# Advaith-Sajeev/LiDAR-Vision-VQA

Hardware: NVIDIA B200
Metric: lidar_encoder_sweeps_per_sec (higher is better)
Workload: dtype f32

## Files before the change

### lidar_vision_vqa_b200/csrc/scatter.cu

```cuda
#include <cuda_fp16.h>

#include <cstdlib>

#include "common.cuh"

namespace pillars {

namespace {

constexpr int kThreads = 256;

__global__ void k_build_cell_row(const void *__restrict__ coords, int coords_float, int64_t m,
                                 const int32_t *__restrict__ m_dev, int nb, int nx, int ny, int nz,
                                 int32_t *__restrict__ cell_row)
{
    const int64_t i = static_cast<int64_t>(blockIdx.x) * blockDim.x + threadIdx.x;
    int64_t live = m;
    if (m_dev) live = tmin<int64_t>(m, static_cast<int64_t>(*m_dev));
    if (i >= live) return;
    int b, z, y, x;
    if (coords_float) {
        const float4 c = *reinterpret_cast<const float4 *>(static_cast<const float *>(coords) + i * 4);
        b = static_cast<int>(c.x); z = static_cast<int>(c.y); y = static_cast<int>(c.z); x = static_cast<int>(c.w);
    } else {
        const int4 c = *reinterpret_cast<const int4 *>(static_cast<const int32_t *>(coords) + i * 4);
        b = c.x; z = c.y; y = c.z; x = c.w;
    }
    const int64_t plane = static_cast<int64_t>(nx) * ny * nz;
    const int64_t cell = nz > 1 ? (static_cast<int64_t>(z) * ny + y) * nx + x : static_cast<int64_t>(z) + static_cast<int64_t>(y) * nx + x;
    if (b < 0 || b >= nb || cell < 0 || cell >= plane || x < 0 || x >= nx) return;
    atomicMax(cell_row + static_cast<int64_t>(b) * plane + cell, static_cast<int32_t>(i));
}

__global__ void k_rebase_segments(int32_t *__restrict__ coords, int n_seg, int64_t rows_per_seg, int64_t seg_stride,
                                  const int32_t *__restrict__ seg_counts, int64_t count_stride, int frames_per_seg,
                                  int32_t *__restrict__ overflow)
{
    const int64_t i = static_cast<int64_t>(blockIdx.x) * blockDim.x + threadIdx.x;
    if (i >= rows_per_seg * n_seg) return;
    const int seg = static_cast<int>(i / rows_per_seg);
    const int64_t r = i - seg * rows_per_seg;
    const int32_t cnt = __ldg(seg_counts + static_cast<int64_t>(seg) * count_stride);
    int32_t *b = coords + seg * seg_stride + r * 4;
    if (r < cnt) *b += seg * frames_per_seg;
    else *b = -1;
    if (r == 0 && cnt > rows_per_seg && overflow) *overflow = 1;
}

template <bool VEC, int CPP, bool PIPE>
__global__ void __launch_bounds__(kThreads)
k_scatter_plain(const float *__restrict__ feats, const int32_t *__restrict__ cell_row, int f, int64_t plane,
                int tiles_per_plane, float *__restrict__ bev)
{
    constexpr int kPer = VEC ? 4 : 1;
    const int b = blockIdx.x / tiles_per_plane;
    const int64_t cell0 = static_cast<int64_t>(blockIdx.x % tiles_per_plane) * (blockDim.x * kPer) + threadIdx.x * kPer;
    const bool inb = cell0 < plane;
    int32_t r[kPer];
#pragma unroll
    for (int k = 0; k < kPer; ++k) r[k] = -1;
    if (inb) {
        if (VEC) {
            const int4 v = __ldg(reinterpret_cast<const int4 *>(cell_row + b * plane + cell0));
            r[0] = v.x; r[1 % kPer] = v.y; r[2 % kPer] = v.z; r[3 % kPer] = v.w;
        } else {
            r[0] = __ldg(cell_row + b * plane + cell0);
        }
    }
    bool any = false;
#pragma unroll
    for (int k = 0; k < kPer; ++k) any |= r[k] >= 0;
    float *dst = bev + (static_cast<int64_t>(b) * f) * plane + cell0;
    if (!__any_sync(0xffffffffu, any)) {
        if (inb) {
            if (VEC) {
#pragma unroll 8
                for (int c = 0; c < f; ++c) __stcs(reinterpret_cast<float4 *>(dst + c * plane), make_float4(0.f, 0.f, 0.f, 0.f));
            } else {
                for (int c = 0; c < f; ++c) __stcs(dst + c * plane, 0.f);
            }
        }
        return;
    }
    if (!inb) return;
    if (VEC) {
        constexpr int kV = CPP / 4;
        float4 cur[4][kV], nxt[4][kV];
        auto fetch = [&](float4 (&dstv)[4][kV], int c0) {
#pragma unroll
            for (int k = 0; k < 4; ++k) {
#pragma unroll
                for (int q = 0; q < kV; ++q) dstv[k][q] = make_float4(0.f, 0.f, 0.f, 0.f);
                if (r[k % kPer] >= 0) {
                    const float4 *row = reinterpret_cast<const float4 *>(feats + static_cast<int64_t>(r[k % kPer]) * f + c0);
#pragma unroll
                    for (int q = 0; q < kV; ++q) dstv[k][q] = __ldg(row + q);
                }
            }
        };
        fetch(cur, 0);
        for (int c0 = 0; c0 < f; c0 += CPP) {
            if (PIPE && c0 + CPP < f) fetch(nxt, c0 + CPP);
#pragma unroll
            for (int q = 0; q < kV; ++q) {
                __stcs(reinterpret_cast<float4 *>(dst + (c0 + 4 * q + 0) * plane), make_float4(cur[0][q].x, cur[1][q].x, cur[2][q].x, cur[3][q].x));
                __stcs(reinterpret_cast<float4 *>(dst + (c0 + 4 * q + 1) * plane), make_float4(cur[0][q].y, cur[1][q].y, cur[2][q].y, cur[3][q].y));
                __stcs(reinterpret_cast<float4 *>(dst + (c0 + 4 * q + 2) * plane), make_float4(cur[0][q].z, cur[1][q].z, cur[2][q].z, cur[3][q].z));
                __stcs(reinterpret_cast<float4 *>(dst + (c0 + 4 * q + 3) * plane), make_float4(cur[0][q].w, cur[1][q].w, cur[2][q].w, cur[3][q].w));
            }
            if (c0 + CPP < f) {
                if (PIPE) {
#pragma unroll
                    for (int k = 0; k < 4; ++k)
#pragma unroll
                        for (int q = 0; q < kV; ++q) cur[k][q] = nxt[k][q];
                } else {
                    fetch(cur, c0 + CPP);
                }
            }
        }
    } else {
        for (int c = 0; c < f; ++c) __stcs(dst + c * plane, r[0] >= 0 ? __ldg(feats + static_cast<int64_t>(r[0]) * f + c) : 0.f);
    }
}

__host__ __device__ __forceinline__ int64_t occ_words(int64_t plane) { return (plane + 255) >> 8; }

__device__ __forceinline__ uint32_t occ_prev_word(const uint32_t *__restrict__ occ_prev, int64_t plane, int tiles_per_plane,
                                                  int groups, int tile_major)
{
    if (!occ_prev) return 0xffffffffu;
    const int tile = tile_major ? (blockIdx.x / groups) % tiles_per_plane : blockIdx.x % tiles_per_plane;
    const int b = blockIdx.x / (groups * tiles_per_plane);
    const int64_t word = (static_cast<int64_t>(tile) * blockDim.x + threadIdx.x) >> 5;
    return word < occ_words(plane) ? __ldg(occ_prev + b * occ_words(plane) + word) : 0xffffffffu;
}

__device__ __forceinline__ void stg256(float *p, float a, float b, float c, float d, float e, float f, float g, float h)
{
    asm volatile("st.global.L1::no_allocate.v8.f32 [%0], {%1, %2, %3, %4, %5, %6, %7, %8};" ::"l"(p), "f"(a), "f"(b), "f"(c),
                 "f"(d), "f"(e), "f"(f), "f"(g), "f"(h)
                 : "memory");
}
__device__ __forceinline__ void stg256_cs(float *p, float a, float b, float c, float d, float e, float f, float g, float h)
{
    asm volatile("st.global.cs.v8.f32 [%0], {%1, %2, %3, %4, %5, %6, %7, %8};" ::"l"(p), "f"(a), "f"(b), "f"(c), "f"(d),
                 "f"(e), "f"(f), "f"(g), "f"(h)
                 : "memory");
}

template <bool CS, int CPP>
__global__ void __launch_bounds__(kThreads)
k_scatter_wide(const float *__restrict__ feats, const int32_t *__restrict__ cell_row, int f, int64_t plane,
               int tiles_per_plane, int chan_per_cta, int tile_major, float *__restrict__ bev,
               const uint32_t *__restrict__ occ_prev, uint32_t *__restrict__ occ_next)
{
    const uint32_t prev = occ_prev_word(occ_prev, plane, tiles_per_plane, f / chan_per_cta, tile_major);
    pdl_wait();
    const int groups = f / chan_per_cta;
    int b, tile, cg;
    if (tile_major) {
        cg = blockIdx.x % groups;
        tile = (blockIdx.x / groups) % tiles_per_plane;
        b = blockIdx.x / (groups * tiles_per_plane);
    } else {
        tile = blockIdx.x % tiles_per_plane;
        cg = (blockIdx.x / tiles_per_plane) % groups;
        b = blockIdx.x / (groups * tiles_per_plane);
    }
    const int64_t cell0 = static_cast<int64_t>(tile) * (blockDim.x * 8) + threadIdx.x * 8;
    const bool inb = cell0 < plane;
    int32_t r[8];
#pragma unroll
    for (int k = 0; k < 8; ++k) r[k] = -1;
    if (inb) {
        const int4 *src = reinterpret_cast<const int4 *>(cell_row + b * plane + cell0);
        const int4 v = __ldg(src), w = __ldg(src + 1);
        r[0] = v.x; r[1] = v.y; r[2] = v.z; r[3] = v.w;
        r[4] = w.x; r[5] = w.y; r[6] = w.z; r[7] = w.w;
    }
    bool any = false;
#pragma unroll
    for (int k = 0; k < 8; ++k) any |= r[k] >= 0;
    const int c_begin = cg * chan_per_cta, c_end = c_begin + chan_per_cta;
    float *dst = bev + (static_cast<int64_t>(b) * f) * plane + cell0;
    auto store = [&](float *p, float a, float b2, float c, float d, float e, float f2, float g, float h) {
        if (CS) stg256_cs(p, a, b2, c, d, e, f2, g, h);
        else stg256(p, a, b2, c, d, e, f2, g, h);
    };
    const uint32_t now = __ballot_sync(0xffffffffu, any);
    if (occ_next && cg == 0 && (threadIdx.x & 31) == 0 && inb) occ_next[b * occ_words(plane) + (cell0 >> 8)] = now;
    if (!inb || !(any || ((prev >> (threadIdx.x & 31)) & 1u))) return;
    if (now == 0) {
#pragma unroll 8
        for (int c = c_begin; c < c_end; ++c) store(dst + c * plane, 0.f, 0.f, 0.f, 0.f, 0.f, 0.f, 0.f, 0.f);
        return;
    }
    constexpr int kV = CPP / 4;
    for (int c0 = c_begin; c0 < c_end; c0 += CPP) {
        float4 v[8][kV];
#pragma unroll
        for (int k = 0; k < 8; ++k) {
#pragma unroll
            for (int q = 0; q < kV; ++q) v[k][q] = make_float4(0.f, 0.f, 0.f, 0.f);
            if (r[k] >= 0) {
                const float4 *row = reinterpret_cast<const float4 *>(feats + static_cast<int64_t>(r[k]) * f + c0);
#pragma unroll
                for (int q = 0; q < kV; ++q) v[k][q] = __ldg(row + q);
            }
        }
#pragma unroll
        for (int q = 0; q < kV; ++q) {
            float *d = dst + (c0 + 4 * q) * plane;
            store(d, v[0][q].x, v[1][q].x, v[2][q].x, v[3][q].x, v[4][q].x, v[5][q].x, v[6][q].x, v[7][q].x);
            store(d + plane, v[0][q].y, v[1][q].y, v[2][q].y, v[3][q].y, v[4][q].y, v[5][q].y, v[6][q].y, v[7][q].y);
            store(d + 2 * plane, v[0][q].z, v[1][q].z, v[2][q].z, v[3][q].z, v[4][q].z, v[5][q].z, v[6][q].z, v[7][q].z);
            store(d + 3 * plane, v[0][q].w, v[1][q].w, v[2][q].w, v[3][q].w, v[4][q].w, v[5][q].w, v[6][q].w, v[7][q].w);
        }
    }
}

__device__ __forceinline__ void ldg256_stream(const float *p, float (&v)[8])
{
    asm volatile("ld.global.nc.L1::no_allocate.v8.f32 {%0, %1, %2, %3, %4, %5, %6, %7}, [%8];"
                 : "=f"(v[0]), "=f"(v[1]), "=f"(v[2]), "=f"(v[3]), "=f"(v[4]), "=f"(v[5]), "=f"(v[6]), "=f"(v[7])
                 : "l"(p));
}

__global__ void __launch_bounds__(kThreads)
k_scatter_wide_half(const float *__restrict__ feats, const int32_t *__restrict__ cell_row, int f, int64_t plane,
                    int tiles_per_plane, __half *__restrict__ bev, const uint32_t *__restrict__ occ_prev,
                    uint32_t *__restrict__ occ_next)
{
    const uint32_t prev = occ_prev_word(occ_prev, plane, tiles_per_plane, f >> 3, 0);
    const int groups = f >> 3;
    const int tile = blockIdx.x % tiles_per_plane;
    const int cg = (blockIdx.x / tiles_per_plane) % groups;
    const int b = blockIdx.x / (groups * tiles_per_plane);
    const int64_t cell0 = static_cast<int64_t>(tile) * (blockDim.x * 8) + threadIdx.x * 8;
    const bool inb = cell0 < plane;
    int32_t r[8];
#pragma unroll
    for (int k = 0; k < 8; ++k) r[k] = -1;
    if (inb) {
        const int4 *src = reinterpret_cast<const int4 *>(cell_row + b * plane + cell0);
        const int4 v = __ldg(src), w = __ldg(src + 1);
        r[0] = v.x; r[1] = v.y; r[2] = v.z; r[3] = v.w;
        r[4] = w.x; r[5] = w.y; r[6] = w.z; r[7] = w.w;
    }
    bool any = false;
#pragma unroll
    for (int k = 0; k < 8; ++k) any |= r[k] >= 0;
    const int c0 = cg * 8;
    __half *dst = bev + (static_cast<int64_t>(b) * f + c0) * plane + cell0;
    const uint32_t now = __ballot_sync(0xffffffffu, any);
    if (occ_next && cg == 0 && (threadIdx.x & 31) == 0 && inb) occ_next[b * occ_words(plane) + (cell0 >> 8)] = now;
    const uint32_t pair = (now | prev) | (((now | prev) >> 1) & 0x55555555u) | (((now | prev) & 0x55555555u) << 1);
    if (!inb || !((pair >> (threadIdx.x & 31)) & 1u)) return;
    if (now == 0) {
#pragma unroll
        for (int c = 0; c < 8; ++c) __stcs(reinterpret_cast<uint4 *>(dst + c * plane), make_uint4(0u, 0u, 0u, 0u));
        return;
    }
    float v[8][8];
#pragma unroll
    for (int k = 0; k < 8; ++k) {
#pragma unroll
        for (int c = 0; c < 8; ++c) v[k][c] = 0.f;
        if (r[k] >= 0) ldg256_stream(feats + static_cast<int64_t>(r[k]) * f + c0, v[k]);
    }
#pragma unroll
    for (int c = 0; c < 8; ++c) {
        uint4 o;
        __half2 h;
        h = __floats2half2_rn(v[0][c], v[1][c]); o.x = *reinterpret_cast<uint32_t *>(&h);
        h = __floats2half2_rn(v[2][c], v[3][c]); o.y = *reinterpret_cast<uint32_t *>(&h);
        h = __floats2half2_rn(v[4][c], v[5][c]); o.z = *reinterpret_cast<uint32_t *>(&h);
        h = __floats2half2_rn(v[6][c], v[7][c]); o.w = *reinterpret_cast<uint32_t *>(&h);
        *reinterpret_cast<uint4 *>(dst + c * plane) = o;
    }
}

}

cudaError_t launch_build_cell_row(const void *coords, bool coords_float, int64_t m, const int32_t *m_dev, int nb, int nx,
                                  int ny, int nz, int32_t *cell_row, cudaStream_t st)
{
    cudaError_t err = cudaMemsetAsync(cell_row, 0xFF, sizeof(int32_t) * static_cast<size_t>(nb) * nx * ny * nz, st);
    note_launch();
    if (err != cudaSuccess || m == 0) return err;
    const unsigned blocks = static_cast<unsigned>((m + kThreads - 1) / kThreads);
    k_build_cell_row<<<blocks, kThreads, 0, st>>>(coords, coords_float ? 1 : 0, m, m_dev, nb, nx, ny, nz, cell_row);
    note_launch();
    return cudaGetLastError();
}

cudaError_t launch_rebase_segments(int32_t *coords, int n_seg, int64_t rows_per_seg, int64_t seg_stride,
                                   const int32_t *seg_counts, int64_t count_stride, int frames_per_seg, int32_t *overflow,
                                   cudaStream_t st)
{
    const int64_t total = rows_per_seg * n_seg;
    if (total == 0) return cudaSuccess;
    k_rebase_segments<<<static_cast<unsigned>((total + kThreads - 1) / kThreads), kThreads, 0, st>>>(
        coords, n_seg, rows_per_seg, seg_stride, seg_counts, count_stride, frames_per_seg, overflow);
    note_launch();
    return cudaGetLastError();
}

cudaError_t launch_scatter_half(const float *feats, const int32_t *cell_row, int nb, int f, int nx, int ny, void *bev,
                                cudaStream_t st, const uint32_t *occ_prev, uint32_t *occ_next)
{
    const int64_t plane = static_cast<int64_t>(nx) * ny;
    if (nb == 0 || plane == 0 || f == 0) return cudaSuccess;
    if (plane % 8 != 0 || f % 8 != 0 || reinterpret_cast<uintptr_t>(bev) % 16 != 0 ||
        reinterpret_cast<uintptr_t>(feats) % 32 != 0)
        return cudaErrorInvalidValue;
    const int bs = 128;
    const int tpp = static_cast<int>((plane + bs * 8 - 1) / (bs * 8));
    const unsigned grid = static_cast<unsigned>(nb) * tpp * (f / 8);
    k_scatter_wide_half<<<grid, bs, 0, st>>>(feats, cell_row, f, plane, tpp, static_cast<__half *>(bev), occ_prev, occ_next);
    note_launch();
    return cudaGetLastError();
}
cudaError_t launch_scatter(const float *feats, const int32_t *cell_row, int nb, int f, int nx, int ny, float *bev,
                           int variant, cudaStream_t st, const uint32_t *occ_prev, uint32_t *occ_next)
{
    const int64_t plane = static_cast<int64_t>(nx) * ny;
    if (nb == 0 || plane == 0 || f == 0) return cudaSuccess;
    const bool vec_ok = (plane % 4 == 0) && (reinterpret_cast<uintptr_t>(bev) % 16 == 0) &&
                        (reinterpret_cast<uintptr_t>(feats) % 16 == 0) && (f % 8 == 0);
    const bool wide_ok = vec_ok && (plane % 8 == 0) && (reinterpret_cast<uintptr_t>(bev) % 32 == 0);
    if (variant != 1 && wide_ok) {
        constexpr int bs = 128, chan = 8;
        const int tpp = static_cast<int>((plane + bs * 8 - 1) / (bs * 8));
        const unsigned grid = static_cast<unsigned>(nb) * tpp * (f / chan);
        static const bool cs = getenv("PILLARS_SCATTER_CS") != nullptr;
        const cudaError_t err = cs ? launch_pdl(k_scatter_wide<true, 8>, dim3(grid), dim3(bs), 0, st, feats, cell_row, f, plane,
                                                tpp, chan, 0, bev, occ_prev, occ_next)
                                   : launch_pdl(k_scatter_wide<false, 8>, dim3(grid), dim3(bs), 0, st, feats, cell_row, f,
                                                plane, tpp, chan, 0, bev, occ_prev, occ_next);
        if (err != cudaSuccess) return err;
        note_launch();
        return cudaGetLastError();
    }
    if (occ_next) {
        const cudaError_t err = cudaMemsetAsync(occ_next, 0xFF, sizeof(uint32_t) * nb * occ_words(plane), st);
        if (err != cudaSuccess) return err;
        note_launch();
    }
    if (vec_ok) {
        const int tpp = static_cast<int>((plane + kThreads * 4 - 1) / (kThreads * 4));
        k_scatter_plain<true, 8, false><<<static_cast<unsigned>(nb) * tpp, kThreads, 0, st>>>(feats, cell_row, f, plane, tpp, bev);
    } else {
        const int tpp = static_cast<int>((plane + kThreads - 1) / kThreads);
        k_scatter_plain<false, 8, false><<<static_cast<unsigned>(nb) * tpp, kThreads, 0, st>>>(feats, cell_row, f, plane, tpp, bev);
    }
    note_launch();
    return cudaGetLastError();
}

}
```

Measured before the change: 89500.

## Add compacted sparse scatter kernel driven by occupancy bitmaps

Adds a sparse scatter kernel that is used whenever a previous occupancy bitmap is available. Each warp reads one bitmap word and ballots which 8-cell groups are occupied now or were occupied before, then compacts those groups into shared memory. The block only loops over that dirty work across all channel chunks, instead of launching a dense grid of tiles per channel group that mostly exit early. The dense kernels drop their occ_prev early-exit logic, and the new kernel adds a shared-memory compaction step plus a block-wide sync.

```diff
diff --git a/lidar_vision_vqa_b200/csrc/scatter.cu b/lidar_vision_vqa_b200/csrc/scatter.cu
--- a/lidar_vision_vqa_b200/csrc/scatter.cu
+++ b/lidar_vision_vqa_b200/csrc/scatter.cu
@@ -126,16 +126,6 @@
 
 __host__ __device__ __forceinline__ int64_t occ_words(int64_t plane) { return (plane + 255) >> 8; }
 
-__device__ __forceinline__ uint32_t occ_prev_word(const uint32_t *__restrict__ occ_prev, int64_t plane, int tiles_per_plane,
-                                                  int groups, int tile_major)
-{
-    if (!occ_prev) return 0xffffffffu;
-    const int tile = tile_major ? (blockIdx.x / groups) % tiles_per_plane : blockIdx.x % tiles_per_plane;
-    const int b = blockIdx.x / (groups * tiles_per_plane);
-    const int64_t word = (static_cast<int64_t>(tile) * blockDim.x + threadIdx.x) >> 5;
-    return word < occ_words(plane) ? __ldg(occ_prev + b * occ_words(plane) + word) : 0xffffffffu;
-}
-
 __device__ __forceinline__ void stg256(float *p, float a, float b, float c, float d, float e, float f, float g, float h)
 {
     asm volatile("st.global.L1::no_allocate.v8.f32 [%0], {%1, %2, %3, %4, %5, %6, %7, %8};" ::"l"(p), "f"(a), "f"(b), "f"(c),
@@ -152,10 +142,8 @@
 template <bool CS, int CPP>
 __global__ void __launch_bounds__(kThreads)
 k_scatter_wide(const float *__restrict__ feats, const int32_t *__restrict__ cell_row, int f, int64_t plane,
-               int tiles_per_plane, int chan_per_cta, int tile_major, float *__restrict__ bev,
-               const uint32_t *__restrict__ occ_prev, uint32_t *__restrict__ occ_next)
-{
-    const uint32_t prev = occ_prev_word(occ_prev, plane, tiles_per_plane, f / chan_per_cta, tile_major);
+               int tiles_per_plane, int chan_per_cta, int tile_major, float *__restrict__ bev, uint32_t *__restrict__ occ_next)
+{
     pdl_wait();
     const int groups = f / chan_per_cta;
     int b, tile, cg;
@@ -190,7 +178,7 @@
     };
     const uint32_t now = __ballot_sync(0xffffffffu, any);
     if (occ_next && cg == 0 && (threadIdx.x & 31) == 0 && inb) occ_next[b * occ_words(plane) + (cell0 >> 8)] = now;
-    if (!inb || !(any || ((prev >> (threadIdx.x & 31)) & 1u))) return;
+    if (!inb) return;
     if (now == 0) {
 #pragma unroll 8
         for (int c = c_begin; c < c_end; ++c) store(dst + c * plane, 0.f, 0.f, 0.f, 0.f, 0.f, 0.f, 0.f, 0.f);
@@ -229,10 +217,8 @@
 
 __global__ void __launch_bounds__(kThreads)
 k_scatter_wide_half(const float *__restrict__ feats, const int32_t *__restrict__ cell_row, int f, int64_t plane,
-                    int tiles_per_plane, __half *__restrict__ bev, const uint32_t *__restrict__ occ_prev,
-                    uint32_t *__restrict__ occ_next)
-{
-    const uint32_t prev = occ_prev_word(occ_prev, plane, tiles_per_plane, f >> 3, 0);
+                    int tiles_per_plane, __half *__restrict__ bev, uint32_t *__restrict__ occ_next)
+{
     const int groups = f >> 3;
     const int tile = blockIdx.x % tiles_per_plane;
     const int cg = (blockIdx.x / tiles_per_plane) % groups;
@@ -255,8 +241,7 @@
     __half *dst = bev + (static_cast<int64_t>(b) * f + c0) * plane + cell0;
     const uint32_t now = __ballot_sync(0xffffffffu, any);
     if (occ_next && cg == 0 && (threadIdx.x & 31) == 0 && inb) occ_next[b * occ_words(plane) + (cell0 >> 8)] = now;
-    const uint32_t pair = (now | prev) | (((now | prev) >> 1) & 0x55555555u) | (((now | prev) & 0x55555555u) << 1);
-    if (!inb || !((pair >> (threadIdx.x & 31)) & 1u)) return;
+    if (!inb) return;
     if (now == 0) {
 #pragma unroll
         for (int c = 0; c < 8; ++c) __stcs(reinterpret_cast<uint4 *>(dst + c * plane), make_uint4(0u, 0u, 0u, 0u));
@@ -281,6 +266,93 @@
     }
 }
 
+constexpr int kSparseWarps = 4;
+
+template <bool HALF>
+__global__ void __launch_bounds__(kSparseWarps * 32)
+k_scatter_sparse(const float *__restrict__ feats, const int32_t *__restrict__ cell_row, int f, int64_t plane,
+                 int spans_per_plane, void *__restrict__ bev, const uint32_t *__restrict__ occ_prev,
+                 uint32_t *__restrict__ occ_next)
+{
+    constexpr int kGroups = kSparseWarps * 32;
+    __shared__ int4 s_rows[2 * kGroups];
+    __shared__ int32_t s_cell[kGroups];
+    __shared__ int s_count[kSparseWarps];
+    const int lane = threadIdx.x & 31, warp = threadIdx.x >> 5;
+    const int b = blockIdx.x / spans_per_plane;
+    const int64_t words = occ_words(plane);
+    const int64_t span_word = static_cast<int64_t>(blockIdx.x % spans_per_plane) * kSparseWarps;
+    const int64_t word = span_word + warp;
+    const uint32_t prev = word < words ? __ldg(occ_prev + b * words + word) : 0u;
+    pdl_wait();
+    const int64_t cell0 = word * 256 + lane * 8;
+    const bool inb = cell0 < plane;
+    int4 v = make_int4(-1, -1, -1, -1), w = v;
+    if (inb) {
+        const int4 *src = reinterpret_cast<const int4 *>(cell_row + b * plane + cell0);
+        v = __ldg(src);
+        w = __ldg(src + 1);
+    }
+    const bool any = (v.x & v.y & v.z & v.w & w.x & w.y & w.z & w.w) >= 0;
+    const uint32_t now = __ballot_sync(0xffffffffu, any);
+    if (lane == 0 && word < words) occ_next[b * words + word] = now;
+    uint32_t dirty = now | prev;
+    if (HALF) dirty |= ((dirty >> 1) & 0x55555555u) | ((dirty & 0x55555555u) << 1);
+    dirty &= __ballot_sync(0xffffffffu, inb);
+    if ((dirty >> lane) & 1u) {
+        const int s = warp * 32 + __popc(dirty & ((1u << lane) - 1u));
+        s_rows[2 * s] = v;
+        s_rows[2 * s + 1] = w;
+        s_cell[s] = static_cast<int>(cell0 - span_word * 256);
+    }
+    const int n = __popc(dirty);
+    if (lane == 0) s_count[warp] = n;
+    __syncthreads();
+    int off[kSparseWarps];
+    off[0] = 0;
+#pragma unroll
+    for (int k = 1; k < kSparseWarps; ++k) off[k] = off[k - 1] + s_count[k - 1];
+    const int total = off[kSparseWarps - 1] + s_count[kSparseWarps - 1];
+    const int items = total * (f >> 3);
+    const int64_t span_base = static_cast<int64_t>(b) * f * plane + span_word * 256;
+    for (int i = threadIdx.x; i < items; i += blockDim.x) {
+        const int chunk = i / total, g = i - chunk * total;
+        int s = g;
+#pragma unroll
+        for (int k = 1; k < kSparseWarps; ++k)
+            if (g >= off[k]) s = k * 32 + g - off[k];
+        const int4 v = s_rows[2 * s], w = s_rows[2 * s + 1];
+        const int r[8] = {v.x, v.y, v.z, v.w, w.x, w.y, w.z, w.w};
+        const int c0 = chunk * 8;
+        float x[8][8];
+#pragma unroll
+        for (int k = 0; k < 8; ++k) {
+#pragma unroll
+            for (int c = 0; c < 8; ++c) x[k][c] = 0.f;
+            if (r[k] >= 0) ldg256_stream(feats + static_cast<int64_t>(r[k]) * f + c0, x[k]);
+        }
+        const int64_t at = span_base + static_cast<int64_t>(c0) * plane + s_cell[s];
+        if (HALF) {
+            __half *dst = static_cast<__half *>(bev) + at;
+#pragma unroll
+            for (int c = 0; c < 8; ++c) {
+                uint4 o;
+                __half2 h;
+                h = __floats2half2_rn(x[0][c], x[1][c]); o.x = *reinterpret_cast<uint32_t *>(&h);
+                h = __floats2half2_rn(x[2][c], x[3][c]); o.y = *reinterpret_cast<uint32_t *>(&h);
+                h = __floats2half2_rn(x[4][c], x[5][c]); o.z = *reinterpret_cast<uint32_t *>(&h);
+                h = __floats2half2_rn(x[6][c], x[7][c]); o.w = *reinterpret_cast<uint32_t *>(&h);
+                *reinterpret_cast<uint4 *>(dst + c * plane) = o;
+            }
+        } else {
+            float *dst = static_cast<float *>(bev) + at;
+#pragma unroll
+            for (int c = 0; c < 8; ++c)
+                stg256(dst + c * plane, x[0][c], x[1][c], x[2][c], x[3][c], x[4][c], x[5][c], x[6][c], x[7][c]);
+        }
+    }
+}
+
 }
 
 cudaError_t launch_build_cell_row(const void *coords, bool coords_float, int64_t m, const int32_t *m_dev, int nb, int nx,
@@ -303,6 +375,18 @@
     if (total == 0) return cudaSuccess;
     k_rebase_segments<<<static_cast<unsigned>((total + kThreads - 1) / kThreads), kThreads, 0, st>>>(
         coords, n_seg, rows_per_seg, seg_stride, seg_counts, count_stride, frames_per_seg, overflow);
+    note_launch();
+    return cudaGetLastError();
+}
+
+template <bool HALF>
+cudaError_t launch_scatter_sparse(const float *feats, const int32_t *cell_row, int nb, int f, int64_t plane, void *bev,
+                                  cudaStream_t st, const uint32_t *occ_prev, uint32_t *occ_next)
+{
+    const int spp = static_cast<int>((occ_words(plane) + kSparseWarps - 1) / kSparseWarps);
+    const cudaError_t err = launch_pdl(k_scatter_sparse<HALF>, dim3(static_cast<unsigned>(nb) * spp), dim3(kSparseWarps * 32),
+                                       0, st, feats, cell_row, f, plane, spp, bev, occ_prev, occ_next);
+    if (err != cudaSuccess) return err;
     note_launch();
     return cudaGetLastError();
 }
@@ -315,10 +399,11 @@
     if (plane % 8 != 0 || f % 8 != 0 || reinterpret_cast<uintptr_t>(bev) % 16 != 0 ||
         reinterpret_cast<uintptr_t>(feats) % 32 != 0)
         return cudaErrorInvalidValue;
+    if (occ_prev) return launch_scatter_sparse<true>(feats, cell_row, nb, f, plane, bev, st, occ_prev, occ_next);
     const int bs = 128;
     const int tpp = static_cast<int>((plane + bs * 8 - 1) / (bs * 8));
     const unsigned grid = static_cast<unsigned>(nb) * tpp * (f / 8);
-    k_scatter_wide_half<<<grid, bs, 0, st>>>(feats, cell_row, f, plane, tpp, static_cast<__half *>(bev), occ_prev, occ_next);
+    k_scatter_wide_half<<<grid, bs, 0, st>>>(feats, cell_row, f, plane, tpp, static_cast<__half *>(bev), occ_next);
     note_launch();
     return cudaGetLastError();
 }
@@ -330,15 +415,17 @@
     const bool vec_ok = (plane % 4 == 0) && (reinterpret_cast<uintptr_t>(bev) % 16 == 0) &&
                         (reinterpret_cast<uintptr_t>(feats) % 16 == 0) && (f % 8 == 0);
     const bool wide_ok = vec_ok && (plane % 8 == 0) && (reinterpret_cast<uintptr_t>(bev) % 32 == 0);
+    if (variant != 1 && wide_ok && occ_prev && reinterpret_cast<uintptr_t>(feats) % 32 == 0)
+        return launch_scatter_sparse<false>(feats, cell_row, nb, f, plane, bev, st, occ_prev, occ_next);
     if (variant != 1 && wide_ok) {
         constexpr int bs = 128, chan = 8;
         const int tpp = static_cast<int>((plane + bs * 8 - 1) / (bs * 8));
         const unsigned grid = static_cast<unsigned>(nb) * tpp * (f / chan);
         static const bool cs = getenv("PILLARS_SCATTER_CS") != nullptr;
         const cudaError_t err = cs ? launch_pdl(k_scatter_wide<true, 8>, dim3(grid), dim3(bs), 0, st, feats, cell_row, f, plane,
-                                                tpp, chan, 0, bev, occ_prev, occ_next)
+                                                tpp, chan, 0, bev, occ_next)
                                    : launch_pdl(k_scatter_wide<false, 8>, dim3(grid), dim3(bs), 0, st, feats, cell_row, f,
-                                                plane, tpp, chan, 0, bev, occ_prev, occ_next);
+                                                plane, tpp, chan, 0, bev, occ_next);
         if (err != cudaSuccess) return err;
         note_launch();
         return cudaGetLastError();
```

Result: faster. 107,000, median of 6 (+19.5%).
